# huakunyang/SummerTTS

Hardware: AMD Instinct MI355X
Metric: audio samples/sec (acoustic model + vocoder, phoneme ids -> int16 PCM on host), single_speaker_fast-shaped synthetic blob (higher is better)
Workload: dtype f32 (decoder trunk convs AND the reverse flow's WaveNet convs (wn_flow.hip, one-utterance calls): fp32 operands as 2 fp16 terms = 22-23 of their 24 mantissa bits, 3 fp16 MFMA products per fp32 product, f32 accumulation -- measured error in `parity`, same tolerance as the exact-fp32 leg; batches addi

## Files before the change

### include/summertts_hip.h

```cpp
#ifndef SUMMERTTS_HIP_H_
#define SUMMERTTS_HIP_H_

#include <stdint.h>

#ifdef __cplusplus
extern "C" {
#endif

typedef struct sts_engine sts_engine;

enum {
    STS_OK = 0,
    STS_EINVAL = -1,
    STS_EMODEL = -2,
    STS_EDEVICE = -3,
    STS_ESTATE = -4
};

int sts_create(const float* blob, int64_t blob_bytes, int device, sts_engine** out);
void sts_destroy(sts_engine* e);

int sts_speaker_num(const sts_engine* e);

typedef struct sts_model_info {
// ... 23 lines not shown

int sts_run_batch(sts_engine* e, int32_t B, const int32_t* const* ids, const int32_t* n, const int32_t* sid,
                  const float* length_scale, int32_t* n_out, int64_t* total_out);
int sts_set_host_pcm(sts_engine* e, int enable);
int sts_copy_pcm_device(sts_engine* e, void* device_dst, int64_t capacity_samples);
int sts_copy_pcm_host(sts_engine* e, int16_t* host_dst, int64_t capacity_samples);
int sts_pcm_host_view(sts_engine* e, const int16_t** pcm, int64_t* count);

int sts_set_forced_durations(sts_engine* e, const int32_t* dur, int64_t count);
int sts_set_noise(sts_engine* e, float noise_scale, float noise_scale_w, uint64_t seed);
int sts_get_noise(const sts_engine* e, float* noise_scale, float* noise_scale_w, uint64_t* seed);
int sts_set_output_rate(sts_engine* e, int32_t rate);
int sts_get_output_rate(const sts_engine* e);
int sts_resample_table(int32_t in_rate, int32_t out_rate, int32_t* P, int32_t* Q, int32_t* taps, float* table, int64_t capacity_floats);
#define STS_LOUD_OFF 0
#define STS_LOUD_MEASURE 1
#define STS_LOUD_NORMALIZE 2
typedef struct sts_loudness { float lufs; float peak; float gain; int32_t blocks; } sts_loudness;
int sts_set_loudness(sts_engine* e, int mode, float target_lufs, float peak_dbfs);
int sts_get_loudness_mode(const sts_engine* e, int* mode, float* target_lufs, float* peak_dbfs);
int sts_get_loudness(sts_engine* e, sts_loudness* out, int64_t capacity);
int sts_kweight_coeffs(int32_t rate, double coeffs[10]);
int sts_loudness_measure(int device, const float* x, const int64_t* lengths, int32_t B, int32_t rate,
                         float target_lufs, float peak_dbfs, sts_loudness* out);
#define STS_LIMITER_OFF 0
#define STS_LIMITER_ON 1
typedef struct sts_limiter_stats { float gain; float min_gain; float peak_out; int32_t limited; } sts_limiter_stats;
int sts_set_limiter(sts_engine* e, int mode, float gain_db, float ceiling_dbfs, float lookahead_ms);
int sts_get_limiter_mode(const sts_engine* e, int* mode, float* gain_db, float* ceiling_dbfs, float* lookahead_ms);
int sts_get_limiter(sts_engine* e, sts_limiter_stats* out, int64_t capacity);
int sts_limiter_design(int32_t rate, float gain_db, float ceiling_dbfs, float lookahead_ms, int32_t* H, double* c, double* G);
int sts_limiter_apply(int device, const float* x, const int64_t* lengths, int32_t B, int32_t rate, float gain_db, float ceiling_dbfs,
                      float lookahead_ms, float* y, int16_t* pcm, sts_limiter_stats* stats);
int sts_set_record_taps(sts_engine* e, int enable);
int sts_get_tap(sts_engine* e, const char* name, float** data, int32_t* channels, int64_t* length);
int sts_get_durations(sts_engine* e, int32_t* dur, int64_t capacity);
int sts_set_conv_mode(sts_engine* e, int mode);
int sts_set_conv_math(sts_engine* e, int mode);

enum { STS_DBG_ATTN_BLOCK_MIN_WGS = 1,
       STS_DBG_TAIL_FUSED = 14 ,
       STS_DBG_UPS_ROWPH = 15 ,
       STS_DBG_CHAIN_STREAMS = 13 ,
       STS_DBG_H2P = 11 ,
       STS_DBG_H2P_TILE = 12 ,
       STS_DBG_MEMO_CLEAR = 10 ,
       STS_DBG_PCM_DIRECT = 9 ,
       STS_DBG_DDS_TAIL = 8 ,
       STS_DBG_ATTN_REG = 7 ,
       STS_DBG_LAUNCH_AHEAD = 6 ,
       STS_DBG_FLOW_FUSED = 5  };
enum { STS_DBG_STREAM_RETRY_STEP = 16, STS_DBG_STREAM_DIRECT = 17 };
enum { STS_DBG_POISON = 18 };
int sts_debug_set(sts_engine* e, int key, int value);

typedef struct sts_profile {
    float ms_text_encoder, ms_duration, ms_flow, ms_decoder, ms_total_device;
    float ms_decoder_mfma;
    int32_t decoder_mfma_launches;
    double flops_text_encoder, flops_duration, flops_flow, flops_decoder;
    double flops_decoder_mfma;
    double bytes_decoder_min;
    int64_t frames, samples, phonemes;
    double flops_decoder_mfma_executed;
    double bytes_text_encoder, bytes_duration, bytes_flow;
    float ms_sync_wait_host;
    double flops_decoder_bf16_issued;
    int64_t conv_math_fallbacks;
    int32_t conv_math_pinned;
    int32_t launch_ahead;
    int64_t launch_ahead_misses;
    float us_host_setup;
    float us_host_enqueue;
    float us_host_tail;
    int64_t poison_bytes;
} sts_profile;
int sts_set_profiling(sts_engine* e, int enable);
#define STS_ABI_VERSION 13
int sts_abi_version(void);
int sts_build_flags(void);
int sts_get_profile(const sts_engine* e, sts_profile* p);
int sts_get_profile_ex(const sts_engine* e, void* p, int64_t size_bytes);

int sts_debug_conv1d(int device, const float* x, int32_t Cin, int32_t L, const float* w, const float* bias,
                     int32_t Cout, int32_t k, int32_t pad, int32_t dil, int32_t stride_transposed,
                     int32_t depthwise, float in_slope, int32_t in_act, int mode, float** y, int32_t* Lout);

int sts_debug_conv1d_bench(int device, const float* x, int32_t Cin, int32_t L, const float* w, const float* bias,
                           int32_t Cout, int32_t k, int32_t pad, int32_t dil, int32_t stride_transposed,
                           int32_t depthwise, float in_slope, int32_t in_act, int mode, float** y, int32_t* Lout,
                           int32_t iters, float* ms_out);

int sts_debug_conv_h2p(int device, const float* x, int32_t Cin, int32_t L, const float* w, const float* bias, int32_t Cout, int32_t k,
                       int32_t dil, const float* res, float in_slope, float out_slope, int tile, int members, float* y, float* y16,
                       float* yp, int32_t iters, float* ms_out);

int sts_debug_conv_h2w(int device, const float* x, int32_t C, int32_t L, const float* w, const float* bias, int32_t k, int32_t dil, const float* res,
                       float in_slope, float out_slope, int members, float* y, float* y16, int32_t iters, float* ms_out);

void sts_free(void* p);
const char* sts_last_error(void);

int sts_debug_wino_pack(const float* w, int32_t Cout, int32_t k, int32_t Cin, float* out, int64_t out_floats);

typedef struct sts_pool sts_pool;
int sts_pool_create(const float* blob, int64_t blob_bytes, int device, int n_engines, int max_batch, sts_pool** out);
// ... 40 lines not shown
```

### summertts_amd/csrc/capi.hip

```cpp
#include <stdlib.h>
#include <string.h>

#include <algorithm>
#include <new>
#include <string>
#include <vector>

#include "engine.hpp"

using namespace sts;

struct sts_engine { Engine eng; };

static thread_local std::string g_err;
static int set_err(int code, const std::string& s) { g_err = s; return code; }

extern "C" {

const char* sts_last_error(void) { return g_err.c_str(); }
void sts_free(void* p) { free(p); }

int sts_create(const float* blob, int64_t blob_bytes, int device, sts_engine** out) {
    if (!out) return set_err(STS_EINVAL, "sts_create: null out pointer");
    *out = nullptr;
// ... 118 lines not shown

int sts_stream_halo_frames(const sts_engine* e) {
    if (!e) return set_err(STS_EINVAL, "null engine");
    return e->eng.stream_halo();
}

int sts_set_forced_durations(sts_engine* e, const int32_t* dur, int64_t count) {
    if (!e) return set_err(STS_EINVAL, "null engine");
    if (!dur || count <= 0) { e->eng.have_forced = false; return STS_OK; }
    e->eng.forced_dur.assign(dur, dur + count);
    e->eng.have_forced = true;
    return STS_OK;
}

int sts_set_noise(sts_engine* e, float noise_scale, float noise_scale_w, uint64_t seed) {
    if (!e) return set_err(STS_EINVAL, "null engine");
    if (!noise_scale_valid(noise_scale) || !noise_scale_valid(noise_scale_w)) return set_err(STS_EINVAL, "noise scales must be finite and >= 0");
    e->eng.noise = Engine::Noise{noise_scale, noise_scale_w, seed};
    return STS_OK;
}
int sts_get_noise(const sts_engine* e, float* noise_scale, float* noise_scale_w, uint64_t* seed) {
    if (!e) return set_err(STS_EINVAL, "null engine");
    if (noise_scale) *noise_scale = e->eng.noise.ns;
    if (noise_scale_w) *noise_scale_w = e->eng.noise.nsw;
    if (seed) *seed = e->eng.noise.seed;
    return STS_OK;
}
int sts_set_record_taps(sts_engine* e, int enable) { if (!e) return set_err(STS_EINVAL, "null engine"); e->eng.record_taps = enable != 0; return STS_OK; }
int sts_set_conv_math(sts_engine* e, int mode) {
    if (!e) return set_err(STS_EINVAL, "null engine");
    if (mode < 0 || mode > 3) return set_err(STS_EINVAL, "conv math: 0 = split-bf16 (default), 1 = exact fp32, 2 = split-bf16 wherever eligible, 3 = two-term fp16");
    e->eng.conv_math = mode;
    e->eng.h2_consecutive = 0; e->eng.h2_disabled = false;
    return STS_OK;
}
int sts_set_conv_mode(sts_engine* e, int mode) { if (!e) return set_err(STS_EINVAL, "null engine"); e->eng.conv_mode = mode; return STS_OK; }
int sts_debug_set(sts_engine* e, int key, int value) {
    if (!e) return set_err(STS_EINVAL, "null engine");
    switch (key) {
        case STS_DBG_ATTN_BLOCK_MIN_WGS: if (value < 1) return set_err(STS_EINVAL, "threshold must be >= 1"); e->eng.attn_block_min_wgs = value; return STS_OK;
        case STS_DBG_FLOW_FUSED: e->eng.flow_fused = value != 0; return STS_OK;
        case STS_DBG_LAUNCH_AHEAD: if (value < 0 || value > 2) return set_err(STS_EINVAL, "launch_ahead must be 0, 1 or 2"); if ((value == 2) != (e->eng.launch_ahead == 2)) { e->eng.seen_tf_.clear(); e->eng.seen_order_.clear(); } e->eng.launch_ahead = value; return STS_OK;
        case STS_DBG_H2P: e->eng.h2p = value < 0 ? 0 : (value > 4 ? 4 : value); return STS_OK;
        case STS_DBG_H2P_TILE: e->eng.h2p_tile = value; return STS_OK;
        case STS_DBG_CHAIN_STREAMS: e->eng.chain_streams_dbg = value; return STS_OK;
        case STS_DBG_TAIL_FUSED: e->eng.tail_fused = value != 0; return STS_OK;
        case STS_DBG_UPS_ROWPH: e->eng.ups_rowph = value != 0; return STS_OK;
        case STS_DBG_MEMO_CLEAR: e->eng.seen_tf_.clear(); e->eng.seen_order_.clear(); return STS_OK;
        case STS_DBG_ATTN_REG: e->eng.attn_reg = value != 0; return STS_OK;
        case STS_DBG_DDS_TAIL: e->eng.dds_tail = value != 0; return STS_OK;
        case STS_DBG_PCM_DIRECT: e->eng.pcm_direct = value != 0; return STS_OK;
        case STS_DBG_STREAM_RETRY_STEP: e->eng.stream_retry_step = value < 0 ? -1 : value; return STS_OK;
        case STS_DBG_STREAM_DIRECT: e->eng.stream_direct = value != 0; return STS_OK;
        case STS_DBG_POISON: e->eng.poison = (unsigned)value; return STS_OK;
        default: return set_err(STS_EINVAL, "unknown debug key");
    }
}
int sts_set_host_pcm(sts_engine* e, int enable) { if (!e) return set_err(STS_EINVAL, "null engine"); e->eng.host_pcm = enable != 0; return STS_OK; }
int sts_set_profiling(sts_engine* e, int enable) { if (!e) return set_err(STS_EINVAL, "null engine"); e->eng.profiling = enable == 2 ? 2 : (enable != 0 ? 1 : 0); return STS_OK; }

int sts_abi_version(void) { return STS_ABI_VERSION; }

int sts_set_output_rate(sts_engine* e, int32_t rate) {
    if (!e) return set_err(STS_EINVAL, "null engine");
    const int rc = e->eng.set_output_rate(rate);
    return rc == STS_OK ? STS_OK : set_err(rc, e->eng.error());
}
int sts_get_output_rate(const sts_engine* e) {
    if (!e) return set_err(STS_EINVAL, "null engine");
    return e->eng.out_rate;
}
int sts_resample_table(int32_t in_rate, int32_t out_rate, int32_t* P, int32_t* Q, int32_t* taps, float* table, int64_t capacity_floats) {
    ResampleDesign d;
    if (!resample_design(in_rate, out_rate, &d)) return set_err(STS_EINVAL, "rates must be integers in [8000, 48000] with P = out / gcd(in, out) <= 1024");
    const int64_t need = (int64_t)d.P * 2 * d.K;
    if (table && capacity_floats < need) return set_err(STS_EINVAL, "table capacity below P * taps floats");
    if (P) *P = d.P;
    if (Q) *Q = d.Q;
    if (taps) *taps = 2 * d.K;
    if (table) resample_table(d, in_rate, out_rate, table);
    return STS_OK;
}
int sts_set_loudness(sts_engine* e, int mode, float target_lufs, float peak_dbfs) {
    if (!e) return set_err(STS_EINVAL, "null engine");
    const int rc = e->eng.set_loudness(mode, target_lufs, peak_dbfs);
    return rc == STS_OK ? STS_OK : set_err(rc, e->eng.error());
}
int sts_get_loudness_mode(const sts_engine* e, int* mode, float* target_lufs, float* peak_dbfs) {
    if (!e) return set_err(STS_EINVAL, "null engine");
    if (mode) *mode = e->eng.loud_mode;
    if (target_lufs) *target_lufs = e->eng.loud_target;
    if (peak_dbfs) *peak_dbfs = e->eng.loud_peak;
    return STS_OK;
}
int sts_get_loudness(sts_engine* e, sts_loudness* out, int64_t capacity) {
    if (!e) return set_err(STS_EINVAL, "null engine");
    const int64_t n = (int64_t)e->eng.loud_res.size();
    if (!out) return (int)n;
    if (capacity < n) return set_err(STS_EINVAL, "capacity below the last call's utterance count");
    if (n > 0) memcpy(out, e->eng.loud_res.data(), (size_t)n * sizeof(sts_loudness));
    return (int)n;
}
int sts_kweight_coeffs(int32_t rate, double coeffs[10]) {
    if (!coeffs) return set_err(STS_EINVAL, "null argument");
    if (!kweight_coeffs(rate, coeffs)) return set_err(STS_EINVAL, "rate must be an integer in [8000, 48000]");
    return STS_OK;
// ... 452 lines not shown
```

### summertts_amd/csrc/engine.hip

```cpp
#include "run_ctx.hpp"
#include <time.h>
#include "knobs.hpp"
#include "../../include/tts_logger.h"

#include <algorithm>
#include <chrono>
#include <math.h>
#include <stdlib.h>
#include <string.h>
#include <thread>

namespace sts {

Engine::~Engine() {
    if (stream) (void)hipStreamSynchronize(stream);
    free_model(model);
    if (arenaT_.base) (void)hipFree(arenaT_.base);
    if (arenaF_.base) (void)hipFree(arenaF_.base);
    if (pinned_) (void)hipHostFree(pinned_);
    if (pinned_pcm_) (void)hipHostFree(pinned_pcm_);
    if (d_rs_table) (void)hipFree(d_rs_table);
    if (loud_host_) (void)hipHostFree(loud_host_);
    if (lim_host_) (void)hipHostFree(lim_host_);
    if (ovf_host_) (void)hipHostFree(ovf_host_);
// ... 147 lines not shown
    const bool use_bf3 = conv_mode == 0 && conv_math != 1 && o.tile < 0 && conv_bf3_eligible(a) &&
                         (in_mfma_region_ || conv_math == 2 || conv_bf3_blocks(a) >= 384);
    if (use_bf3 && c.transposed && ups_rowph && a.epi == EPI_STORE && !a.ubias && (a.math == 1 ? c.wh2r : c.wb3r)) {
        a.wb3 = a.math == 1 ? c.wh2r : c.wb3r;
        a.bias = c.bias ? c.bias_r : nullptr;
        a.Cout = a.Cout_pad = c.Cout_pad * c.stride;
        a.rowph = c.stride;
    }
    if (a.nsum >= 2 && !(use_bf3 ? conv_bf3_takes_sum(a) : (!can_mfma && conv_cout1_takes(a)))) {
        const float* r[3] = {x, o.sum1, o.sum2};
        sum_scale(o.sum_dst, r, a.nsum, o.sum_n, cur_);
        a.x = o.sum_dst; a.xs1 = a.xs2 = nullptr; a.nsum = 0;
    }
    if (use_bf3) {
        if (in_mfma_region_) { mfma_flops_ += fl; bf16_exec_ += products() * fl; mfma_launches_++; }
        static const int bt = exp_int("STS_BF3_TILE", -1);
        conv_bf3(a, cur_, bt);
    } else if (can_mfma) {
        if (in_mfma_region_) { mfma_flops_ += fl; mfma_exec_ += fl; mfma_launches_++; }
        conv_mfma(a, cur_, o.tile >= 0 ? o.tile : (conv_mode >= 2 ? conv_mode - 2 : -1));
    } else {
        if (a.kslices > 1 && a.kslice_stride > 0)
            (void)hipMemsetAsync(a.y + a.kslice_stride, 0, (size_t)(a.kslices - 1) * (size_t)a.kslice_stride * sizeof(float), cur_);
        conv_generic(a, cur_);
    }
}

int Engine::pick_kslices(const DConv& c, const Lvl& lout) const {
    if (conv_mode != 0 || c.depthwise || c.transposed || c.Cin < 32) return 1;
    const long tiles = (long)((lout.max_len + 31) / 32) * (c.Cout_pad / 32) * lout.nb;
    const long groups = (long)c.k * (c.Cin_pad / 8);
    int s = 1;
    while (s < 8 && tiles * (s * 2) <= 256 && groups / (s * 2) >= 24) s *= 2;
    return s;
}

void Engine::ln(const DLn& l, const float* a, const float* b, const float* res, float* y, const Lvl& lv, int pre_relu, int post_gelu, int nb, long b_stride) {
    LnArgs g;
    memset(&g, 0, sizeof(g));
    g.a = a; g.a_ld = lv.ld; g.b = b; g.b_ld = lv.ld; g.res = res; g.res_ld = lv.ld; g.y = y; g.y_ld = lv.ld;
    g.nb = nb; g.b_stride = b_stride;
    g.gamma = l.g; g.beta = l.b; g.C = l.C; g.pre_relu = pre_relu; g.post_gelu = post_gelu;
    g.seg = lv.seg; g.B = lv.nb; g.max_len = lv.max_len;
    bytes_[cur_stage_] += 4.0 * (double)l.C * (double)lv.total * (2.0 + (b ? 1.0 : 0.0) + (res ? 1.0 : 0.0));
    layer_norm(g, cur_);
}

float* Engine::dds(const DDds& d, float* h, float* t1, float* t2, const Lvl& lv, const DConv* pre, const float* pre_in, const float* pre_res,
                   const SplineTail* tail, bool* tail_done) {
    if (tail_done) *tail_done = false;
    static const bool no_col = exp_flag("STS_NO_COL_LAYER");
    float* cur = h;
    bool pre_pending = pre != nullptr;
    auto run_pre = [&]() {
        if (!pre_pending) return;
        pre_pending = false;
        const float* in = pre_in;
        if (!in) { (void)hipMemsetAsync(t2, 0, (size_t)lv.total * sizeof(float), cur_); in = t2; }
        ConvOpt oa; oa.epi = EPI_RESADD; oa.res = pre_res;
        conv(*pre, in, lv, h, lv, oa);
    };
    for (int i = 0; i < d.n; i++) {
        const DConv& c = d.sep[i];
        const DConv& pw = d.pw[i];
        if (!no_col && conv_mode != 1 && !pw.depthwise && pw.k == 1 && pw.Cin == pw.Cout && pw.Cin == d.n1[i].C && pw.Cin == d.n2[i].C &&
            pw.Cin_pad == pw.Cin) {
            ColLayerArgs g;
            memset(&g, 0, sizeof(g));
            float* nxt = cur == h ? t1 : h;
            g.x = cur; g.x_ld = lv.ld;
            g.dw_w = c.w; g.dw_b = c.bias; g.dw_k = c.k; g.dw_dil = c.dil; g.dw_pad = c.pad; g.dw_ld = c.Cout_pad;
            g.g1 = d.n1[i].g; g.b1 = d.n1[i].b;
            g.wc = pw.wc; g.bias = pw.bias;
            g.g2 = d.n2[i].g; g.b2 = d.n2[i].b; g.post_gelu = 1;
            g.res = cur; g.res_ld = lv.ld; g.y = nxt; g.y_ld = lv.ld; g.C = pw.Cin;
            g.seg = lv.seg; g.B = lv.nb; g.max_len = lv.max_len;
            if (pre_pending && i == 0 && pre->Cin == 1 && pre->k == 1 && pre->Cout == pw.Cin && !pre->depthwise && pre_res) {
                g.x = pre_res; g.res = pre_res; g.xs_w = pre->w; g.xs_b = pre->bias; g.xr = pre_in;
                if (col_layer_eligible(g)) {
                    pre_pending = false;
                    flops_[cur_stage_] += 2.0 * pre->macs_per_out * (double)lv.total;
                } else { g.x = cur; g.res = cur; g.xs_w = g.xs_b = g.xr = nullptr; }
            }
            run_pre();
            if (tail && tail_done && dds_tail && i == d.n - 1 && tail->proj && tail->proj->k == 1 && !tail->proj->depthwise && tail->proj->Cout == 29 &&
                tail->proj->Cout_pad == 32 && tail->proj->Cin == pw.Cin && tail->proj->Cin_pad == pw.Cin && tail->proj->w && tail->proj->bias) {
                ColLayerArgs gt = g;
                gt.tp_w = tail->proj->w; gt.tp_b = tail->proj->bias; gt.tp_fs = tail->filter_sqrt;
                gt.tp_r0 = tail->r0; gt.tp_r1 = tail->r1; gt.tp_o0 = tail->o0; gt.tp_o1 = tail->o1;
                if (col_layer_eligible(gt)) {
                    flops_[cur_stage_] += 2.0 * (c.macs_per_out + pw.macs_per_out + tail->proj->macs_per_out) * (double)lv.total;
                    bytes_[cur_stage_] += 4.0 * ((double)pw.Cin * lv.total + (double)pw.Cin * pw.Cout + (double)pw.Cin * 32 + 4.0 * lv.total);
                    col_layer(gt, cur_);
                    *tail_done = true;
                    return nxt;
                }
            }
            if (col_layer_eligible(g)) {
                flops_[cur_stage_] += 2.0 * (c.macs_per_out + pw.macs_per_out) * (double)lv.total;
                bytes_[cur_stage_] += 4.0 * ((double)pw.Cin * lv.total * 2.0 + (double)pw.Cin * pw.Cout);
                col_layer(g, cur_);
                cur = nxt;
                continue;
            }
        }
        run_pre();
// ... 1032 lines not shown
```

### summertts_amd/csrc/engine.hpp

```cpp
#pragma once
#include <hip/hip_runtime.h>

#include <deque>
#include <map>
#include <unordered_map>
#include <string>
#include <vector>

#include "../../include/summertts_hip.h"
#include "kernels.hpp"
#include "model.hpp"

namespace sts {

struct Arena {
    char* base = nullptr; size_t cap = 0, used = 0; bool measuring = false;
    void* alloc(size_t bytes) {
        size_t a = (used + 255) & ~(size_t)255;
        used = a + bytes;
        if (measuring) return nullptr;
        return base + a;
    }
    template <typename T> T* get(size_t count) { return (T*)alloc(count * sizeof(T)); }
};
// ... 30 lines not shown

struct Tap { std::vector<float> data; int channels = 0; long length = 0; };
constexpr int kNativeRate = 16000;

class Engine {
public:
    ~Engine();
    int init(const float* blob, int64_t bytes, int device);
    int run(int B, const int32_t* const* ids, const int32_t* n, const int32_t* sid, const float* ls, const StreamSpec* ss = nullptr);
    int run_once(int B, const int32_t* const* ids, const int32_t* n, const int32_t* sid, const float* ls, const StreamSpec* ss);
    int run_batch_stream(int B, const int32_t* const* ids, const int32_t* n, const int32_t* sid, const float* ls, int chunk_frames,
                         int (*cb)(void*, int32_t, const int16_t*, int32_t, int32_t), void* user, int32_t* n_total);
    const std::string& error() const { return err_; }

    Model model;
    int device = 0;
    std::vector<int32_t> n_samples;
    int64_t total_samples = 0;
    int16_t* d_pcm = nullptr;
    const int16_t* pcm_hbm() const { return pcm_in_host_ ? nullptr : d_pcm; }
    float host_us_setup_ = 0, host_us_enq_ = 0;
    double host_t0_ = 0, host_t_sync_ = 0;
    bool pcm_in_host_ = false;
    const int16_t* h_pcm = nullptr;
    bool host_pcm = false;
    std::vector<int32_t> durations_h;
    std::map<std::string, Tap> taps;
    sts_profile prof{};
    struct Noise { float ns = 0.f, nsw = 0.f; uint64_t seed = 0; };
    Noise noise;
    std::vector<Noise> noise_utt;
    int out_rate = kNativeRate;
    ResampleDesign rs;
    float* d_rs_table = nullptr;
    bool resampling() const { return out_rate != kNativeRate; }
    long long out_count(long long native) const { return resampling() ? (native * rs.P + rs.Q - 1) / rs.Q : native; }
    int set_output_rate(int rate);
    int stream_halo() const;
    int loud_mode = 0; float loud_target = -16.f, loud_peak = -1.f;
    std::vector<sts_loudness> loud_res;
    int set_loudness(int mode, float target, float peak);
    int lim_mode = 0; float lim_gain_db = 0.f, lim_ceiling = -1.f, lim_ms = 5.f;
    std::vector<sts_limiter_stats> lim_res;
    int set_limiter(int mode, float gain_db, float ceiling_dbfs, float lookahead_ms);
    std::vector<int32_t> forced_dur; bool have_forced = false;
    bool record_taps = false; int profiling = 0;
    int conv_mode = 0;
    int conv_math = 3;
    long h2_fallbacks = 0;
    int h2_consecutive = 0; bool h2_disabled = false;
    double products() const { return conv_math == 3 ? 3.0 : 6.0; }
    int pcm_direct = 1;
    int dds_tail = 1;
    int attn_reg = 1;
    int attn_block_min_wgs = 96;
    int launch_ahead = 1;
    long ahead_misses = 0;
    static constexpr size_t kMemoEntries = 1024;
    std::unordered_map<unsigned long long, long> seen_tf_; std::deque<unsigned long long> seen_order_;
    bool polite_wait = false;
    struct WaitEst { double us = 0.0; long phonemes = 0; };
    WaitEst wait_est_[2][24];
    void nap_before_wait(int which, long phonemes);
    void note_wait(int which, long phonemes, double waited_us, bool was_ready_at_wake);
    int final_sync(long phonemes);
    int ups_rowph = 1;
    int tail_fused = 1;
    int chain_streams_dbg = -1;
    int h2p = 1;
    int h2p_tile = -1;
    int flow_fused = 1;
    int stream_retry_step = -1;
    int stream_direct = 0;
    unsigned poison = 0;
    int64_t poison_bytes_ = 0;
    hipStream_t stream = nullptr;

private:
    int fail(int code, const std::string& msg) { err_ = msg; return code; }
    bool ensure(Arena& a, size_t bytes);
    bool ensure_pinned(size_t bytes);
    void poison_arena(const Arena& a);
    void poison_host16(void* p, size_t samples);
    void poison_host32(void* p, size_t words);
    ConvArgs conv_args(const DConv& c, const float* x, const Lvl& lin, float* y, const Lvl& lout, const ConvOpt& o, double* flops);
    void conv(const DConv& c, const float* x, const Lvl& lin, float* y, const Lvl& lout, const ConvOpt& o);
    void ln(const DLn& l, const float* a, const float* b, const float* res, float* y, const Lvl& lv, int pre_relu, int post_gelu, int nb = 1, long b_stride = 0);
    int pick_kslices(const DConv& c, const Lvl& lout) const;
    struct SplineTail { const DConv* proj; float filter_sqrt; const float* r0; const float* r1; float* o0; float* o1; };
    float* dds(const DDds& d, float* h, float* t1, float* t2, const Lvl& lv, const DConv* pre = nullptr, const float* pre_in = nullptr,
               const float* pre_res = nullptr, const SplineTail* tail = nullptr, bool* tail_done = nullptr);
    struct RunCtx;
    struct ResStage;
    int run_setup(RunCtx& c);
    int run_text_encoder(RunCtx& c);
    int run_durations(RunCtx& c);
    int run_frame_workspace(RunCtx& c);
    int run_flow(RunCtx& c);
    int run_decode(RunCtx& c, int nw, long Wtot, int maxW, int zoff0, int wlen0);
    int decode_end(RunCtx& c, const float* wave, const WinGeom& win, long Wtot, int maxW);
    int wait_frame_counts(RunCtx& c);
    int frame_geometry(RunCtx& c);
    int run_output(RunCtx& c);
    int run_stream_steps(RunCtx& c);
    void tap(const char* name, const float* d, int channels, long ld, long length);
    void stage_begin(int s);
// ... 29 lines not shown
```

### summertts_amd/csrc/kernels.hpp

```cpp
#pragma once
#include <hip/hip_runtime.h>
#include <stdint.h>

namespace sts {

struct SegView {
    const int* off;
    const int* len;
    int scale;
    int extra;
    int ioff, ilen;
};

enum Epilogue : int {
    EPI_STORE = 0,
    EPI_RESADD = 1,
    EPI_SUB = 3,
    EPI_GATE = 4,
    EPI_RESSKIP = 5,
    EPI_TANH_PCM = 6,
};

struct ConvArgs {
    const float* x; long x_ld;
// ... 14 lines not shown
    int epi, epi_flag; float epi_scale; int H;
    int gate_perm;
    SegView in_seg, out_seg;
    int B, max_n;
    int kslices; long kslice_stride;
    const float* wu; int wino_n3, wino_n2;
    const void* wb3;
    int keep_lo, keep_hi;
    int math; float wscale; unsigned* ovf;
    const float* xs1; const float* xs2; int nsum;
    int rowph;
};

__host__ __device__ inline void wino_split(int k, int* n3, int* n2) { *n2 = (k % 3 == 0) ? 0 : (k % 3 == 2 ? 1 : 2); *n3 = (k - 2 * *n2) / 3; }
void wino_pack(const float* w, long s_out, long s_tap, long s_in, int Cout, int k, int Cin, int Cin_pad, int Cout_pad, float* dst);
bool conv_wino_eligible(const ConvArgs& a);
void conv_wino(const ConvArgs& a, hipStream_t st);

struct LnArgs {
    const float* a; long a_ld;
    const float* b; long b_ld;
    int nb; long b_stride;
    const float* res; long res_ld;
    float* y; long y_ld;
    const float* gamma; const float* beta;
    int C;
    int pre_relu, post_gelu;
    const float* dw_w; const float* dw_b; int dw_k, dw_dil, dw_pad, dw_ld;
    SegView seg; int B, max_len;
};

struct ColLayerArgs {
    const float* x; long x_ld;
    const float* xs_w; const float* xs_b; const float* xr;
    const float* dw_w; const float* dw_b; int dw_k, dw_dil, dw_pad, dw_ld;
    const float* g1; const float* b1;
    const float* wc; const float* bias;
    const float* add; long add_ld;
    const float* g2; const float* b2; int post_gelu;
    const float* res; long res_ld;
    float* y; long y_ld;
    int C;
    SegView seg; int B, max_len;
    const float* tp_w; const float* tp_b;
    float tp_fs;
    const float* tp_r0; const float* tp_r1;
    float* tp_o0; float* tp_o1;
};
bool col_layer_eligible(const ColLayerArgs& a);
bool col_layer_width_ok(int C);
void col_layer_pack(const float* w, int C, float* dst);
void col_layer(const ColLayerArgs& a, hipStream_t st);

struct ColProjArgs {
    const int* ids; const float* emb; int vocab; float emb_scale;
    const float* a; long a_ld; const float* bp; long b_ld; int nb; long b_stride;
    const float* gamma; const float* beta;
    float* x_out; long x_ld;
    const float* wc; const float* bias; int Cout, npass;
    float* y; long y_ld;
    int C;
    SegView seg; int B, max_len;
};
bool col_proj_eligible(const ColProjArgs& a);
void col_proj(const ColProjArgs& a, hipStream_t st);
void col_proj_pack(const float* w, int C, int Cout, float* dst);

struct AttnArgs {
    const float* q; const float* k; const float* v; float* o; long ld;
    const float* relk; const float* relv;
    int kc, px, win, nheads;
    SegView seg; int B, max_len;
    int block_min_wgs;
    int attn_reg;
};


struct FlowLayerArgs {
    SegView seg; int B, max_len; long tot;
    int H, half, G, Cg, k, halo;
    int layer;
    const float* x0; long x0_ld; const float* pend; int pend_n; long pend_stride; float* x0_out; long x0_out_ld;
    const void* w_pre; const float* b_pre; float s_pre;
    const float* h_in; const float* part_in; int part_n; long part_stride;
    float* h_out;
    float* part_out;
    float* macc; long macc_stride; int macc_init;
    const void* w_gate; const float* b_gate; float s_gate;
    const float* ubias; int ubias_ld;
    const void* w_c; float s_c; int rows_c, rows_res;
    const float* b_res; const float* b_m;
    unsigned* ovf;
};
struct FlowFinishArgs {
    SegView seg; int B, max_len; int half;
    const float* src; long src_ld; float* dst; long dst_ld;
    const float* macc; int n; long macc_stride;
};
bool flow_layer_shape_ok(int H, int half, int k, int dil, int n_layers);
int flow_layer_groups(int H);
void flow_layer(const FlowLayerArgs& a, hipStream_t st);
void flow_finish(const FlowFinishArgs& a, hipStream_t st);

bool conv_mfma_eligible(const ConvArgs& a);
void conv_mfma(const ConvArgs& a, hipStream_t st, int tile = -1);
constexpr int kMaxGroup = 4;
// ... 142 lines not shown
```

### summertts_amd/csrc/knobs.hpp

```cpp
#pragma once
#include <stdlib.h>

namespace sts {
#ifdef STS_EXPERIMENTS
inline const char* exp_env(const char* name) { return getenv(name); }
#else
inline const char* exp_env(const char*) { return nullptr; }
#endif
inline int exp_int(const char* name, int dflt) { const char* v = exp_env(name); return v ? atoi(v) : dflt; }
inline bool exp_flag(const char* name) { return exp_env(name) != nullptr; }
}
```

### summertts_amd/engine.py

```python
from __future__ import annotations

import ctypes as C
import os
import subprocess
from typing import Dict, List, Optional, Sequence

import numpy as np

_HERE = os.path.dirname(os.path.abspath(__file__))
LIB_PATH = os.environ.get("SUMMERTTS_HIP_LIB") or os.path.join(_HERE, "lib", "libsummertts_hip.so")
CSRC = os.path.join(_HERE, "csrc")


def build_library(verbose: bool = False) -> str:
    subprocess.run(["make", "-C", CSRC, "-j8"], check=True, stdout=None if verbose else subprocess.DEVNULL)
    return LIB_PATH


class ModelInfo(C.Structure):
    _fields_ = [("is_multi_speaker", C.c_int32), ("lang_type", C.c_int32), ("dur_pred_type", C.c_int32),
                ("dec_type", C.c_int32), ("vocab", C.c_int32), ("hidden", C.c_int32), ("inter_channels", C.c_int32),
                ("speaker_num", C.c_int32), ("gin_channels", C.c_int32), ("samples_per_frame", C.c_int32),
                ("sample_rate", C.c_int32), ("blob_floats_consumed", C.c_int64)]

# ... 330 lines not shown

    def set_output_rate(self, rate: int):
        _check(self.lib, self.lib.sts_set_output_rate(self.h, int(rate)))

    def output_rate(self) -> int:
        return int(self.lib.sts_get_output_rate(self.h))

    def set_loudness(self, mode: int, target_lufs: float = -16.0, peak_dbfs: float = -1.0):
        _check(self.lib, self.lib.sts_set_loudness(self.h, int(mode), float(target_lufs), float(peak_dbfs)))

    def loudness_mode(self):
        m, t, p = C.c_int(), C.c_float(), C.c_float()
        _check(self.lib, self.lib.sts_get_loudness_mode(self.h, C.byref(m), C.byref(t), C.byref(p)))
        return m.value, t.value, p.value

    def loudness(self) -> np.ndarray:
        n = self.lib.sts_get_loudness(self.h, None, 0)
        if n < 0:
            _check(self.lib, n)
        out = np.zeros(n, LOUDNESS_DTYPE)
        if n:
            rc = self.lib.sts_get_loudness(self.h, out.ctypes.data, n)
            if rc < 0:
                _check(self.lib, rc)
        return out

    def set_limiter(self, mode: int, gain_db: float = 0.0, ceiling_dbfs: float = -1.0, lookahead_ms: float = 5.0):
        _check(self.lib, self.lib.sts_set_limiter(self.h, int(mode), float(gain_db), float(ceiling_dbfs), float(lookahead_ms)))

    def limiter_mode(self):
        m, g, c, l = C.c_int(), C.c_float(), C.c_float(), C.c_float()
        _check(self.lib, self.lib.sts_get_limiter_mode(self.h, C.byref(m), C.byref(g), C.byref(c), C.byref(l)))
        return m.value, g.value, c.value, l.value

    def limiter(self) -> np.ndarray:
        n = self.lib.sts_get_limiter(self.h, None, 0)
        if n < 0:
            _check(self.lib, n)
        out = np.zeros(n, LIMITER_DTYPE)
        if n:
            rc = self.lib.sts_get_limiter(self.h, out.ctypes.data, n)
            if rc < 0:
                _check(self.lib, rc)
        return out

    def set_conv_math(self, mode):
        m = {"bf16x3": 0, "f32": 1, "bf16x3_all": 2, "f16x2": 3}.get(mode, mode)
        _check(self.lib, self.lib.sts_set_conv_math(self.h, int(m)))

    def set_conv_mode(self, mode: int):
        _check(self.lib, self.lib.sts_set_conv_mode(self.h, mode))

    def debug_set(self, key: str, value: int):
        _check(self.lib, self.lib.sts_debug_set(self.h, {"attn_block_min_wgs": 1, "flow_fused": 5, "launch_ahead": 6, "attn_reg": 7, "dds_tail": 8, "pcm_direct": 9, "memo_clear": 10, "h2p": 11, "h2p_tile": 12, "chain_streams": 13, "tail_fused": 14, "ups_rowph": 15, "stream_retry_step": 16, "stream_direct": 17, "poison": 18}[key], int(value)))

    def set_profiling(self, on):
        _check(self.lib, self.lib.sts_set_profiling(self.h, 2 if on == 2 else (1 if on else 0)))

    def profile(self) -> dict:
        p = Profile()
        _check(self.lib, self.lib.sts_get_profile_ex(self.h, C.byref(p), C.sizeof(p)))
        return p.as_dict()

    def tap(self, name: str) -> np.ndarray:
        ptr = C.POINTER(C.c_float)()
        ch, ln = C.c_int32(), C.c_int64()
        _check(self.lib, self.lib.sts_get_tap(self.h, name.encode(), C.byref(ptr), C.byref(ch), C.byref(ln)))
        a = np.ctypeslib.as_array(ptr, shape=(ch.value, ln.value)).copy()
        self.lib.sts_free(ptr)
        return a

    def durations(self, total_phonemes: int) -> np.ndarray:
        d = np.zeros(total_phonemes, np.int32)
        _check(self.lib, self.lib.sts_get_durations(self.h, d.ctypes.data, d.size))
        return d

    def close(self):
        if getattr(self, "h", None) is not None and self.h:
            self.lib.sts_destroy(self.h)
            self.h = None

    def __del__(self):
        try:
            self.close()
        except Exception:
            pass


def debug_conv1d(x: np.ndarray, w: np.ndarray, bias: Optional[np.ndarray], pad: int, dil: int = 1,
                 stride_transposed: int = 0, depthwise: bool = False, in_slope: float = 0.0, in_act: int = 0,
                 mode: int = 0, device: int = 0, iters: int = 0):
    lib = load_library()
    x = np.ascontiguousarray(x, np.float32)
    w = np.ascontiguousarray(w, np.float32)
    cout, k = w.shape[0], w.shape[1]
    b = None if bias is None else np.ascontiguousarray(bias, np.float32)
    y = C.POINTER(C.c_float)()
    lout = C.c_int32()
    ms = C.c_float(0.0)
    _check(lib, lib.sts_debug_conv1d_bench(device, x.ctypes.data, x.shape[0], x.shape[1], w.ctypes.data,
                                           None if b is None else b.ctypes.data, cout, k, pad, dil, stride_transposed,
                                           1 if depthwise else 0, in_slope, in_act, mode, C.byref(y), C.byref(lout),
                                           iters, C.byref(ms)))
    out = np.ctypeslib.as_array(y, shape=(cout, lout.value)).copy()
    lib.sts_free(y)
    return (out, float(ms.value)) if iters > 0 else out

# ... 267 lines not shown
```

Measured before the change: 66.79 million.

## Fuse whole DDS conv stack into one windowed kernel with halo recompute

Adds a kernel that runs all layers of the dilated depth-separable conv stack (depthwise conv, layernorm, GELU, pointwise MFMA conv, layernorm, GELU, residual) for a 16-column strip in a single launch. It keeps activations in shared memory with a halo window and recomputes overlapping edges. It can also fold in the preceding 1-channel projection and the spline projection tail. This removes per-layer launches and global-memory round trips in the duration predictor and flow stages, at the cost of redundant halo compute and heavy shared-memory use. It is enabled by default when the grid is small.

```diff
diff --git a/include/summertts_hip.h b/include/summertts_hip.h
--- a/include/summertts_hip.h
+++ b/include/summertts_hip.h
@@ -99,6 +99,7 @@
        STS_DBG_FLOW_FUSED = 5  };
 enum { STS_DBG_STREAM_RETRY_STEP = 16, STS_DBG_STREAM_DIRECT = 17 };
 enum { STS_DBG_POISON = 18 };
+enum { STS_DBG_DDS_STACK = 19 };
 int sts_debug_set(sts_engine* e, int key, int value);
 
 typedef struct sts_profile {
diff --git a/summertts_amd/csrc/capi.hip b/summertts_amd/csrc/capi.hip
--- a/summertts_amd/csrc/capi.hip
+++ b/summertts_amd/csrc/capi.hip
@@ -194,6 +194,7 @@
         case STS_DBG_PCM_DIRECT: e->eng.pcm_direct = value != 0; return STS_OK;
         case STS_DBG_STREAM_RETRY_STEP: e->eng.stream_retry_step = value < 0 ? -1 : value; return STS_OK;
         case STS_DBG_STREAM_DIRECT: e->eng.stream_direct = value != 0; return STS_OK;
+        case STS_DBG_DDS_STACK: if (value < 0 || value > 2) return set_err(STS_EINVAL, "dds_stack must be 0, 1 or 2"); e->eng.dds_stack = value; return STS_OK;
         case STS_DBG_POISON: e->eng.poison = (unsigned)value; return STS_OK;
         default: return set_err(STS_EINVAL, "unknown debug key");
     }
diff --git a/summertts_amd/csrc/dds_stack.hip b/summertts_amd/csrc/dds_stack.hip
--- /dev/null
+++ b/summertts_amd/csrc/dds_stack.hip
@@ -0,0 +1,232 @@
+#include "kernels.hpp"
+#include "devmath.hpp"
+
+namespace sts {
+
+typedef float f32x4 __attribute__((ext_vector_type(4)));
+
+namespace {
+constexpr int kW = 48;
+enum { P_DW0 = 0, P_DWB = 3, P_G1 = 4, P_B1 = 5, P_BIAS = 6, P_G2 = 7, P_B2 = 8, P_ROWS = 9 };
+
+__device__ __forceinline__ int ds_seg_start(const SegView& s, int b) { return (s.off ? s.off[b] : s.ioff) * s.scale + b * s.extra; }
+__device__ __forceinline__ int ds_seg_len(const SegView& s, int b) { return (s.off ? s.len[b] : s.ilen) * s.scale + s.extra; }
+
+__device__ __forceinline__ float ds_param(const DdsStackLayer& L, int r, int c) {
+    switch (r) {
+        case 0: case 1: case 2: return r < L.dw_k ? L.dw_w[(size_t)r * L.dw_ld + c] : 0.f;
+        case P_DWB: return L.dw_b ? L.dw_b[c] : 0.f;
+        case P_G1: return L.g1[c];
+        case P_B1: return L.b1[c];
+        case P_BIAS: return L.bias ? L.bias[c] : 0.f;
+        case P_G2: return L.g2[c];
+        default: return L.b2[c];
+    }
+}
+}
+
+template <int NSUB, bool TAIL>
+__global__ __launch_bounds__(64 * NSUB) void dds_stack_kernel(DdsStackArgs a) {
+    constexpr int C = 16 * NSUB, KQ = C / 4, CG = 4 * NSUB, NT = 64 * NSUB;
+    constexpr int KH = KQ > 16 ? 12 : KQ;
+    static_assert(KQ % KH == 0 && (C * kW) % NT == 0 && NT == 4 * C, "window and strip tiling");
+    __shared__ __attribute__((aligned(16))) float buf[2][C * kW];
+    __shared__ float par[kDdsStackMaxLayers][P_ROWS][C];
+    __shared__ float red1[2][NSUB][16], red2[2][NSUB][16];
+    __shared__ float tp[TAIL ? 32 * 16 : 1], wb[TAIL ? 32 : 1];
+    const int b = blockIdx.y;
+    const int len = ds_seg_len(a.seg, b);
+    const int n0 = blockIdx.x * 16;
+    if (n0 >= len) return;
+    const size_t base = (size_t)ds_seg_start(a.seg, b);
+    const int tid = threadIdx.x, lane = tid & 63, wave = tid >> 6;
+    const int col = lane & 15, quad = lane >> 4;
+    const int cg = tid >> 4;
+    const int org = n0 - 16;
+    const int row0 = wave * 16 + quad * 4;
+
+    {
+        float v[C * kW / NT];
+#pragma unroll
+        for (int t = 0; t < C * kW / NT; t++) {
+            const int idx = tid + t * NT, c = idx / kW, p = org + (idx - c * kW);
+            float xv = 0.f;
+            if (p >= 0 && p < len) {
+                xv = a.x[(size_t)c * a.x_ld + base + p];
+                if (a.xs_w)
+                    xv = __fadd_rn(__fadd_rn(__fmul_rn(a.xs_w[c], a.xr ? a.xr[base + p] : 0.f), a.xs_b ? a.xs_b[c] : 0.f), xv);
+            }
+            v[t] = xv;
+        }
+#pragma unroll
+        for (int t = 0; t < C * kW / NT; t++) buf[0][tid + t * NT] = v[t];
+    }
+    f32x4 af[KQ / 4], afn[KQ / 4];
+    auto load_strip = [&](const float* wc, f32x4 (&dst)[KQ / 4]) {
+        const f32x4* wp = reinterpret_cast<const f32x4*>(wc) + (size_t)wave * (KQ / 4) * 64 + lane;
+#pragma unroll
+        for (int i = 0; i < KQ / 4; i++) dst[i] = wp[(size_t)i * 64];
+    };
+    load_strip(a.L[0].wc, af);
+    for (int l = 0; l < a.n; l++) {
+        const DdsStackLayer& L = a.L[l];
+        for (int r = tid / C; r < P_ROWS; r += 4) par[l][r][tid % C] = ds_param(L, r, tid % C);
+    }
+    __syncthreads();
+
+    for (int l = 0; l < a.n; l++) {
+        const DdsStackLayer& L = a.L[l];
+        const float* in = buf[l & 1];
+        float* out = buf[(l & 1) ^ 1];
+        const bool last = l == a.n - 1;
+        if (!last) load_strip(a.L[l + 1].wc, afn);
+        else if (TAIL) {
+            const f32x4* twp = reinterpret_cast<const f32x4*>(a.tp_w) + tid;
+            afn[0] = twp[0]; afn[1] = twp[NT];
+        }
+        const int dw_k = L.dw_k, dw_dil = L.dw_dil, dw_pad = L.dw_pad;
+        const int blk0 = a.reach[l] > 0 ? 0 : 1, blk1 = a.reach[l] > 0 ? 3 : 2;
+        for (int blk = blk0; blk < blk1; blk++) {
+            const int lc = blk * 16 + col, pos = org + lc;
+            const bool live = pos >= 0 && pos < len;
+            {
+                float v[4];
+                float s = 0.f, sq = 0.f;
+#pragma unroll
+                for (int i = 0; i < 4; i++) {
+                    const int c = cg + i * CG;
+                    float acc = par[l][P_DWB][c];
+#pragma unroll
+                    for (int j = 0; j < 3; j++) {
+                        const int lq = lc + j * dw_dil - dw_pad, q = pos + j * dw_dil - dw_pad;
+                        const bool ok = live && j < dw_k && q >= 0 && q < len && lq >= 0 && lq < kW;
+                        const float xin = ok ? in[c * kW + lq] : 0.f;
+                        acc += par[l][P_DW0 + j][c] * xin;
+                    }
+                    v[i] = acc; s += acc; sq += acc * acc;
+                }
+                s += __shfl_xor(s, 16, 64); sq += __shfl_xor(sq, 16, 64);
+                s += __shfl_xor(s, 32, 64); sq += __shfl_xor(sq, 32, 64);
+                if (quad == 0) { red1[0][wave][col] = s; red1[1][wave][col] = sq; }
+                __syncthreads();
+                s = 0.f; sq = 0.f;
+#pragma unroll
+                for (int k = 0; k < NSUB; k++) { s += red1[0][k][col]; sq += red1[1][k][col]; }
+                const float mean = s / (float)C;
+                const float var = sq * (float)(1. / (float)C) - mean * mean;
+                const float den = (float)sqrt((double)var + 1e-05);
+#pragma unroll
+                for (int i = 0; i < 4; i++) {
+                    const int c = cg + i * CG;
+                    float o = ((v[i] - mean) / den) * par[l][P_G1][c] + par[l][P_B1][c];
+                    o = gelu_ref(o);
+                    out[c * kW + lc] = live ? o : 0.f;
+                }
+            }
+            __syncthreads();
+
+            f32x4 acc0 = {0.f, 0.f, 0.f, 0.f}, acc1 = {0.f, 0.f, 0.f, 0.f};
+#pragma unroll
+            for (int h0 = 0; h0 < KQ; h0 += KH) {
+                float bq[KH];
+#pragma unroll
+                for (int i = 0; i < KH; i++) bq[i] = out[(4 * (h0 + i) + quad) * kW + lc];
+#pragma unroll
+                for (int i = 0; i < KH; i += 2) {
+                    acc0 = __builtin_amdgcn_mfma_f32_16x16x4f32(af[(h0 + i) / 4][(h0 + i) % 4], bq[i], acc0, 0, 0, 0);
+                    acc1 = __builtin_amdgcn_mfma_f32_16x16x4f32(af[(h0 + i + 1) / 4][(h0 + i + 1) % 4], bq[i + 1], acc1, 0, 0, 0);
+                }
+            }
+
+            float v[4];
+            float s = 0.f, sq = 0.f;
+#pragma unroll
+            for (int r = 0; r < 4; r++) { v[r] = 0.f + ((acc0[r] + acc1[r]) + par[l][P_BIAS][row0 + r]); s += v[r]; sq += v[r] * v[r]; }
+            s += __shfl_xor(s, 16, 64); sq += __shfl_xor(sq, 16, 64);
+            s += __shfl_xor(s, 32, 64); sq += __shfl_xor(sq, 32, 64);
+            if (quad == 0) { red2[0][wave][col] = s; red2[1][wave][col] = sq; }
+            __syncthreads();
+            s = 0.f; sq = 0.f;
+#pragma unroll
+            for (int k = 0; k < NSUB; k++) { s += red2[0][k][col]; sq += red2[1][k][col]; }
+            const float mean = s / (float)C;
+            const float var = sq * (float)(1. / (float)C) - mean * mean;
+            const float den = (float)sqrt((double)var + 1e-05);
+#pragma unroll
+            for (int r = 0; r < 4; r++) {
+                float o = ((v[r] - mean) / den) * par[l][P_G2][row0 + r] + par[l][P_B2][row0 + r];
+                o = gelu_ref(o);
+                o = (live ? in[(row0 + r) * kW + lc] : 0.f) + o;
+                out[(row0 + r) * kW + lc] = live ? o : 0.f;
+                if (!TAIL && last && live) a.y[(size_t)(row0 + r) * a.y_ld + base + pos] = o;
+            }
+        }
+        __syncthreads();
+        if (!last) {
+#pragma unroll
+            for (int i = 0; i < KQ / 4; i++) af[i] = afn[i];
+        }
+        if (TAIL && last) {
+            float* wl = buf[l & 1];
+            const bool live = n0 + col < len;
+            float t_in = 0.f, t_keep = 0.f;
+            if (tid < 16 && live) { t_in = a.tp_r1 ? a.tp_r1[base + n0 + tid] : 0.f; t_keep = a.tp_r0 ? a.tp_r0[base + n0 + tid] : 0.f; }
+            reinterpret_cast<f32x4*>(wl)[tid] = afn[0]; reinterpret_cast<f32x4*>(wl)[tid + NT] = afn[1];
+            if (tid < 32) wb[tid] = tid < 29 ? a.tp_b[tid] : 0.f;
+            __syncthreads();
+            for (int j = tid >> 4; j < 32; j += 4 * NSUB) {
+                float acc = 0.f;
+#pragma unroll 8
+                for (int c = 0; c < C; c++) acc += wl[c * 32 + j] * out[c * kW + 16 + col];
+                acc += wb[j];
+                tp[j * 16 + col] = j < 29 ? rq_spline_param(j, acc, a.tp_fs) : 0.f;
+            }
+            __syncthreads();
+            if (tid < 16 && live) {
+                float t[29];
+#pragma unroll
+                for (int j = 0; j < 29; j++) t[j] = tp[j * 16 + tid];
+                a.tp_o0[base + n0 + tid] = rq_spline_inverse_t(t_in, t);
+                a.tp_o1[base + n0 + tid] = t_keep;
+            }
+        }
+    }
+}
+
+bool dds_stack_width_ok(int C) { return C == 32 || C == 64 || C == 192; }
+
+bool dds_stack_eligible(DdsStackArgs& a) {
+    if (!dds_stack_width_ok(a.C) || a.n < 1 || a.n > kDdsStackMaxLayers || !a.x) return false;
+    int reach = 0;
+    for (int l = a.n - 1; l >= 0; l--) {
+        const DdsStackLayer& L = a.L[l];
+        if (!L.dw_w || !L.g1 || !L.b1 || !L.wc || !L.g2 || !L.b2) return false;
+        if ((L.dw_k != 1 && L.dw_k != 3) || L.dw_dil < 1 || L.dw_pad != L.dw_dil * (L.dw_k - 1) / 2) return false;
+        a.reach[l] = reach;
+        reach += L.dw_pad;
+    }
+    if (reach > 16) return false;
+    if (a.tp_w) {
+        if (!a.tp_b || !a.tp_o0 || !a.tp_o1 || a.tp_o0 == a.tp_r0 || a.tp_o0 == a.tp_r1 || a.tp_o1 == a.tp_r1) return false;
+    } else if (!a.y || a.y == a.x) return false;
+    return a.max_len > 0 && a.B > 0;
+}
+
+void dds_stack(const DdsStackArgs& a, hipStream_t st) {
+    const dim3 grid((a.max_len + 15) / 16, a.B);
+    if (a.tp_w) {
+        switch (a.C) {
+            case 32: hipLaunchKernelGGL((dds_stack_kernel<2, true>), grid, dim3(128), 0, st, a); break;
+            case 64: hipLaunchKernelGGL((dds_stack_kernel<4, true>), grid, dim3(256), 0, st, a); break;
+            default: hipLaunchKernelGGL((dds_stack_kernel<12, true>), grid, dim3(768), 0, st, a); break;
+        }
+        return;
+    }
+    switch (a.C) {
+        case 32: hipLaunchKernelGGL((dds_stack_kernel<2, false>), grid, dim3(128), 0, st, a); break;
+        case 64: hipLaunchKernelGGL((dds_stack_kernel<4, false>), grid, dim3(256), 0, st, a); break;
+        default: hipLaunchKernelGGL((dds_stack_kernel<12, false>), grid, dim3(768), 0, st, a); break;
+    }
+}
+
+}
diff --git a/summertts_amd/csrc/engine.hip b/summertts_amd/csrc/engine.hip
--- a/summertts_amd/csrc/engine.hip
+++ b/summertts_amd/csrc/engine.hip
@@ -223,6 +223,50 @@
     static const bool no_col = exp_flag("STS_NO_COL_LAYER");
     float* cur = h;
     bool pre_pending = pre != nullptr;
+    if (!no_col && conv_mode != 1 && dds_stack != 0 && d.n >= 1 && d.n <= kDdsStackMaxLayers &&
+        (dds_stack == 2 || (long)((lv.max_len + 15) / 16) * lv.nb <= kDdsStackMaxBlocks)) {
+        DdsStackArgs g;
+        memset(&g, 0, sizeof(g));
+        const int C = d.pw[0].Cin;
+        bool ok = true;
+        for (int i = 0; i < d.n && ok; i++) {
+            const DConv& c = d.sep[i];
+            const DConv& pw = d.pw[i];
+            ok = !pw.depthwise && pw.k == 1 && pw.Cin == C && pw.Cout == C && d.n1[i].C == C && d.n2[i].C == C && pw.Cin_pad == C && pw.wc != nullptr;
+            DdsStackLayer& L = g.L[i];
+            L.dw_w = c.w; L.dw_b = c.bias; L.dw_k = c.k; L.dw_dil = c.dil; L.dw_pad = c.pad; L.dw_ld = c.Cout_pad;
+            L.g1 = d.n1[i].g; L.b1 = d.n1[i].b; L.wc = pw.wc; L.bias = pw.bias; L.g2 = d.n2[i].g; L.b2 = d.n2[i].b;
+        }
+        g.n = d.n; g.C = C; g.x = h; g.x_ld = lv.ld; g.y = t1; g.y_ld = lv.ld;
+        g.seg = lv.seg; g.B = lv.nb; g.max_len = lv.max_len;
+        if (pre) {
+            ok = ok && pre->Cin == 1 && pre->k == 1 && pre->Cout == C && !pre->depthwise && pre_res;
+            g.x = pre_res; g.xs_w = pre->w; g.xs_b = pre->bias; g.xr = pre_in;
+        }
+        const bool with_tail = tail && tail_done && dds_tail && tail->proj && tail->proj->k == 1 && !tail->proj->depthwise && tail->proj->Cout == 29 &&
+                               tail->proj->Cout_pad == 32 && tail->proj->Cin == C && tail->proj->Cin_pad == C && tail->proj->w && tail->proj->bias;
+        if (with_tail) {
+            g.tp_w = tail->proj->w; g.tp_b = tail->proj->bias; g.tp_fs = tail->filter_sqrt;
+            g.tp_r0 = tail->r0; g.tp_r1 = tail->r1; g.tp_o0 = tail->o0; g.tp_o1 = tail->o1;
+        }
+        if (ok && dds_stack_eligible(g)) {
+            if (pre) flops_[cur_stage_] += 2.0 * pre->macs_per_out * (double)lv.total;
+            for (int i = 0; i < d.n; i++) {
+                const DConv& c = d.sep[i];
+                const DConv& pw = d.pw[i];
+                if (with_tail && i == d.n - 1) {
+                    flops_[cur_stage_] += 2.0 * (c.macs_per_out + pw.macs_per_out + tail->proj->macs_per_out) * (double)lv.total;
+                    bytes_[cur_stage_] += 4.0 * ((double)pw.Cin * lv.total + (double)pw.Cin * pw.Cout + (double)pw.Cin * 32 + 4.0 * lv.total);
+                } else {
+                    flops_[cur_stage_] += 2.0 * (c.macs_per_out + pw.macs_per_out) * (double)lv.total;
+                    bytes_[cur_stage_] += 4.0 * ((double)pw.Cin * lv.total * 2.0 + (double)pw.Cin * pw.Cout);
+                }
+            }
+            sts::dds_stack(g, cur_);
+            if (with_tail) *tail_done = true;
+            return t1;
+        }
+    }
     auto run_pre = [&]() {
         if (!pre_pending) return;
         pre_pending = false;
diff --git a/summertts_amd/csrc/engine.hpp b/summertts_amd/csrc/engine.hpp
--- a/summertts_amd/csrc/engine.hpp
+++ b/summertts_amd/csrc/engine.hpp
@@ -106,6 +106,7 @@
     double products() const { return conv_math == 3 ? 3.0 : 6.0; }
     int pcm_direct = 1;
     int dds_tail = 1;
+    int dds_stack = 1;
     int attn_reg = 1;
     int attn_block_min_wgs = 96;
     int launch_ahead = 1;
diff --git a/summertts_amd/csrc/kernels.hpp b/summertts_amd/csrc/kernels.hpp
--- a/summertts_amd/csrc/kernels.hpp
+++ b/summertts_amd/csrc/kernels.hpp
@@ -90,6 +90,27 @@
 void col_layer_pack(const float* w, int C, float* dst);
 void col_layer(const ColLayerArgs& a, hipStream_t st);
 
+constexpr int kDdsStackMaxLayers = 4;
+struct DdsStackLayer {
+    const float* dw_w; const float* dw_b; int dw_k, dw_dil, dw_pad, dw_ld;
+    const float* g1; const float* b1;
+    const float* wc; const float* bias;
+    const float* g2; const float* b2;
+};
+struct DdsStackArgs {
+    const float* x; long x_ld;
+    const float* xs_w; const float* xs_b; const float* xr;
+    int n; DdsStackLayer L[kDdsStackMaxLayers];
+    int reach[kDdsStackMaxLayers];
+    float* y; long y_ld;
+    int C;
+    SegView seg; int B, max_len;
+    const float* tp_w; const float* tp_b; float tp_fs;
+    const float* tp_r0; const float* tp_r1; float* tp_o0; float* tp_o1;
+};
+bool dds_stack_eligible(DdsStackArgs& a);
+void dds_stack(const DdsStackArgs& a, hipStream_t st);
+
 struct ColProjArgs {
     const int* ids; const float* emb; int vocab; float emb_scale;
     const float* a; long a_ld; const float* bp; long b_ld; int nb; long b_stride;
diff --git a/summertts_amd/csrc/knobs.hpp b/summertts_amd/csrc/knobs.hpp
--- a/summertts_amd/csrc/knobs.hpp
+++ b/summertts_amd/csrc/knobs.hpp
@@ -2,6 +2,7 @@
 #include <stdlib.h>
 
 namespace sts {
+constexpr int kDdsStackMaxBlocks = 256;
 #ifdef STS_EXPERIMENTS
 inline const char* exp_env(const char* name) { return getenv(name); }
 #else
diff --git a/summertts_amd/engine.py b/summertts_amd/engine.py
--- a/summertts_amd/engine.py
+++ b/summertts_amd/engine.py
@@ -406,7 +406,7 @@
         _check(self.lib, self.lib.sts_set_conv_mode(self.h, mode))
 
     def debug_set(self, key: str, value: int):
-        _check(self.lib, self.lib.sts_debug_set(self.h, {"attn_block_min_wgs": 1, "flow_fused": 5, "launch_ahead": 6, "attn_reg": 7, "dds_tail": 8, "pcm_direct": 9, "memo_clear": 10, "h2p": 11, "h2p_tile": 12, "chain_streams": 13, "tail_fused": 14, "ups_rowph": 15, "stream_retry_step": 16, "stream_direct": 17, "poison": 18}[key], int(value)))
+        _check(self.lib, self.lib.sts_debug_set(self.h, {"attn_block_min_wgs": 1, "flow_fused": 5, "launch_ahead": 6, "attn_reg": 7, "dds_tail": 8, "pcm_direct": 9, "memo_clear": 10, "h2p": 11, "h2p_tile": 12, "chain_streams": 13, "tail_fused": 14, "ups_rowph": 15, "stream_retry_step": 16, "stream_direct": 17, "poison": 18, "dds_stack": 19}[key], int(value)))
 
     def set_profiling(self, on):
         _check(self.lib, self.lib.sts_set_profiling(self.h, 2 if on == 2 else (1 if on else 0)))
```

Result: slower. 63.31 million (-5.2%).
